# NeSC-IV/sage-icp

Measured on AMD Instinct MI355X. Metric: ICP frames/sec (120k-pt scan vs 1M-pt map), higher is better.
Workload: dtype f64

## Files before the change

### sage-icp_amd/build.py

```python
import concurrent.futures
import hashlib
import os
import subprocess

HERE = os.path.dirname(os.path.abspath(__file__))
SOURCES = ["csrc/kernels.hip", "csrc/sort.hip", "csrc/preprocess.hip", "csrc/dyn_filter.hip", "csrc/deskew.hip",
           "csrc/ingest.hip", "csrc/egress.hip", "csrc/msg.hip", "csrc/keyframe.hip", "csrc/map_update.hip",
           "csrc/map_device.hip", "csrc/capi_run.hip", "csrc/prep.hip", "csrc/capi.hip", "csrc/capi_pipeline.hip",
           "csrc/capi_outputs.hip", "csrc/caller_mem.hip", "csrc/correspond.hip"]
HEADERS = ["csrc/kernels.h", "csrc/dev_buffer.h", "csrc/sageicp_types.h", "csrc/se3_math.h", "csrc/host_map.hpp", "csrc/pipeline.hpp", "csrc/map_update.h", "csrc/egress.h", "csrc/msg.h", "csrc/metrics.hpp", "csrc/robin_order.hpp", "csrc/capi_internal.h", "csrc/prep.h", "csrc/prefetch.h", "csrc/dyn_rules.h", "csrc/probes.h", "csrc/icp_body.h", "csrc/row_shift.h", "csrc/fin_kernel.h", "csrc/loop_kernel.h", "csrc/caller_mem.h", "csrc/outputs.h", "csrc/map_device.h", "csrc/replay_pool.h", "csrc/correspond.h",
           "../include/sageicp.h"]
OUT = os.path.join(HERE, "libsageicp_hip.so")
OBJ_DIR = os.path.join(HERE, "build")

FLAGS = ["--offload-arch=gfx950", "-O3", "-std=c++17", "-fPIC", "-ffp-contract=off",
         "-Wall", "-Wextra"]


def _stamp(extra):
    h = hashlib.sha1(" ".join(FLAGS + list(extra)).encode())
    for f in HEADERS:
        with open(os.path.join(HERE, f), "rb") as fh:
            h.update(fh.read())
    return h.hexdigest()[:16]


def needs_build():
    if not os.path.exists(OUT):
        return True
    t = os.path.getmtime(OUT)
    return any(os.path.getmtime(os.path.join(HERE, f)) > t for f in SOURCES + HEADERS)


# ... 69 lines not shown
```

### sage-icp_amd/csrc/capi_internal.h

```cpp
#pragma once

#include <dlfcn.h>
#include <hip/hip_runtime.h>
#include <rccl/rccl.h>

#include <atomic>
#include <chrono>
#include <cmath>
#include <cstdio>
#include <cstdlib>
#include <cfloat>
#include <limits>
#include <memory>
#include <cstring>
#include <map>
#include <array>
#include <string>
#include <utility>
#include <vector>

#include "../../include/sageicp.h"
#include "dev_buffer.h"
#include "dyn_rules.h"
#include "host_map.hpp"
// ... 83 lines not shown

inline double now_us() {
    using namespace std::chrono;
    return duration<double, std::micro>(steady_clock::now().time_since_epoch()).count();
}

constexpr int kChunkMax = 16;

struct Scratch {
    int device = -1;
    OwnedStream stream;
    DevBuf<Point4> d_frame, d_tgt;
    DevBuf<int32_t> d_nn;
    DevBuf<Point4> d_sorted;
    DevBuf<uint32_t> d_keys, d_vals;
    DevBuf<unsigned char> d_sort_temp;
    size_t sort_cap = 0;
    DevBuf<uint32_t> d_rows;
    DevBuf<uint2> d_prev;
    DevBuf<uint32_t> d_work;
    DevBuf<double> d_partials;
    DevBuf<long long> d_acc;
    DevBuf<LoopShared> d_loop;
    unsigned long long go_word = 0;
    OwnedStream stream2;
    std::vector<uint32_t> cu_mask;
    OwnedEvent ev_solve;
    unsigned long long loop_epoch = 0;
    int num_cus = 0;
    int cu_share_i = 0, cu_share_k = 1;
    int loop_cooldown = 0;
    int loop_derate = 0;
    uint64_t calls_single_launch = 0, calls_per_iteration = 0, calls_chained = 0;
    uint32_t loop_timeouts = 0;
    int last_fallback = 0;
    DevBuf<unsigned long long> d_cand;
    DevBuf<IcpState> d_state;
    PinnedBuf<IcpState> h_state;
    PinnedBuf<IcpProgress, hipHostMallocMapped | hipHostMallocCoherent> h_prog;
    IcpProgress *d_prog = nullptr;
    std::vector<OwnedEvent> events;
    DevBuf<int32_t> d_by_query;
    DevBuf<uint32_t> d_corr_counts;
    DevBuf<unsigned long long> d_corr_words;
    PinnedBuf<unsigned long long> h_corr_words;

// ... 69 lines not shown
        return SAGEICP_OK;
    }
    int reserve_nn(size_t n) {
        if (n > d_nn.capacity()) HIPCHK(d_nn.reserve(n + n / 4 + 1024));
        return SAGEICP_OK;
    }
    int reserve_sort(size_t n) {
        if (n <= sort_cap) return SAGEICP_OK;
        sort_cap = 0;
        const size_t cap = n + n / 4 + 1024;
        HIPCHK(d_sorted.reserve(cap));
        HIPCHK(d_rows.reserve(cap * kRowWords));
        HIPCHK(d_prev.reserve(cap));
#ifdef SAGE_NN_TIMING
        HIPCHK(d_work.reserve(cap));
#endif
        HIPCHK(d_cand.reserve(2 * cap));
        HIPCHK(d_keys.reserve(2 * cap));
        HIPCHK(d_vals.reserve(2 * cap));
        HIPCHK(d_sort_temp.reserve(sort_temp_bytes(static_cast<int>(cap))));
        sort_cap = cap;
        return SAGEICP_OK;
    }
    int reserve_correspond(size_t n) {
        if (n > d_by_query.capacity()) HIPCHK(d_by_query.reserve(n + n / 4 + 1024));
        const size_t words = 2 * static_cast<size_t>(correspond_blocks(static_cast<int>(n)));
        if (words > d_corr_counts.capacity()) HIPCHK(d_corr_counts.reserve(words + words / 4 + 16));
        if (!d_corr_words) HIPCHK(d_corr_words.reserve(2));
        if (!h_corr_words) HIPCHK(h_corr_words.reserve(2));
        return SAGEICP_OK;
    }
    int reserve_partials(size_t blocks) {
        if (blocks > d_partials.capacity() / kNumSums) HIPCHK(d_partials.reserve((blocks + blocks / 4 + 256) * kNumSums));
        return SAGEICP_OK;
    }
    int reserve_events(size_t iterations) {
        while (events.size() < 5 * iterations) {
            OwnedEvent e;
            HIPCHK(e.create(hipEventDefault));
            events.push_back(std::move(e));
        }
        return SAGEICP_OK;
    }
};


// ... 91 lines not shown
```

### sage-icp_amd/csrc/capi_run.hip

```cpp
#include "capi_internal.h"

#include <condition_variable>
#include <mutex>
#include <thread>

namespace sageicp_impl {

Rccl g_rccl;
static std::mutex g_rccl_mu;


int load_rccl() {
    std::lock_guard<std::mutex> lk(g_rccl_mu);
    if (g_rccl.h) return SAGEICP_OK;
    const char *names[] = {"librccl.so.1", "librccl.so", "/opt/rocm/lib/librccl.so.1"};
    void *h = nullptr;
    for (const char *n : names) {
        h = dlopen(n, RTLD_NOW | RTLD_NOLOAD | RTLD_GLOBAL);
        if (h) break;
    }
    for (int i = 0; i < 3 && !h; ++i) h = dlopen(names[i], RTLD_NOW | RTLD_GLOBAL);
    if (!h) return fail(SAGEICP_ERR_RCCL, std::string("cannot load librccl: ") + dlerror());
    g_rccl.GetUniqueId = reinterpret_cast<decltype(g_rccl.GetUniqueId)>(dlsym(h, "ncclGetUniqueId"));
    g_rccl.CommInitRank = reinterpret_cast<decltype(g_rccl.CommInitRank)>(dlsym(h, "ncclCommInitRank"));
// ... 88 lines not shown
    ip.work = sc.d_work.data();
    ip.acc_scale = std::ldexp(1.0, -24 * std::max(acc_shift, std::min(2, std::max(0, env_int("SAGEICP_ACC_SHIFT", 0)))));
    {
        const uint64_t blocks = std::max<uint64_t>(1, (n + 3) / 4);
        int bits = 0;
        while ((1ull << bits) < blocks) ++bits;
        ip.digit_limit = std::ldexp(1.0, std::min(46, 62 - bits));
    }
    ip.counters = nullptr;
    ip.stripe_work = nullptr;
    ip.stripe_order = nullptr;
    const uint64_t qw = 64u >> lw;
    ip.nwaves = static_cast<unsigned>((n + qw - 1) / qw);
#ifdef SAGE_ICP_DELAY_PROBE
    ip.dbg_delay = static_cast<unsigned>(env_int("SAGEICP_DBG_DELAY", 0));
    ip.dbg_repeat = static_cast<unsigned>(env_int("SAGEICP_DBG_REPEAT", 0));
#endif
    return ip;
}

struct LoopPlan {
    int lw, nw, gpw, wgs;
    bool filter;
};
static int loop_wgs_per_cu(const Scratch &sc, int lw, bool filter, int nw, size_t lds) {
    static std::mutex mu;
    static std::map<std::array<long, 5>, int> cache;
    const std::array<long, 5> key{sc.device, lw, filter ? 1 : 0, nw, static_cast<long>(lds)};
    int v;
    {
        std::lock_guard<std::mutex> lk(mu);
        auto it = cache.find(key);
        if (it == cache.end()) it = cache.emplace(key, loop_blocks_per_cu(lw, filter, nw, lds)).first;
        v = it->second;
    }
    return std::min(v, SAGE_LOOP_OCC / ((nw + 3) / 4));
}
static bool plan_loop(const sageicp_map &m, uint64_t n, double sem_th, LoopPlan *out) {
    const Scratch &sc = m.sc;
    const int mode = env_int("SAGEICP_LOOP", 1);
    if (mode == 0 || n == 0 || sc.num_cus < 8) return false;
    const bool sparse = sparse_voxels(m);
    const bool filter = wants_filter(m, n, sem_th);
    const uint64_t cus = static_cast<uint64_t>(sc.num_cus);
    const int env_nw = std::min(kLoopMaxWavesHost, std::max(0, env_int("SAGEICP_LOOP_WAVES", 0)));
    const int env_gpw = std::max(0, env_int("SAGEICP_LOOP_GPW", 0));
    auto groups_at = [n](int l) { return (n + (64u >> l) - 1) / (64u >> l); };
    auto slots = [&](int k) {
        const uint64_t a = static_cast<uint64_t>(k) * cus * 15 / 16;
        int less = 0;
        for (int sh = 1; sh < sc.cu_share_k; sh *= 2) ++less;
        return (less > 0 && k > less) ? std::min(a, static_cast<uint64_t>(k - less) * cus) : a;
    };
    auto round32 = [](uint64_t w) { return std::max<uint64_t>(32, (w + 31) / 32 * 32); };
    auto countable = [](uint64_t wgs, uint64_t gpw, int lw) {
        return wgs / kLoopReplicas <= 255 && (wgs / kLoopReplicas) * gpw * ((64u >> lw) / 4u) <= 8192;
    };
    auto one_pass = [&](int lw, int nw, LoopPlan *pl) {
        const uint64_t wgs = round32((groups_at(lw) + nw - 1) / nw);
        const size_t lds = loop_lds_bytes(lw, nw, nw);
        const int k = loop_wgs_per_cu(sc, lw, filter, nw, lds);
        if (k < 1 || wgs + 32ull * static_cast<uint64_t>(sc.loop_derate) > slots(k) || !countable(wgs, nw, lw)) return false;
        *pl = LoopPlan{lw, nw, nw, static_cast<int>(wgs), filter};
        return true;
    };
    auto multi_pass = [&](int lw, LoopPlan *pl) {
        const uint64_t groups = groups_at(lw);
        int best = -1;
        const int order[] = {4, 8, 7, 6, 5, 3, 2, 1};
        for (int nw : order) {
            if (env_nw && nw != env_nw) continue;
            if (!env_nw && nw < 4) continue;
            for (int k = SAGE_LOOP_OCC / ((nw + 3) / 4); k >= 1; --k) {
                if (static_cast<uint64_t>(k) * cus < 34) break;
                uint64_t cap = slots(k) / 32 * 32;
                cap = cap > 32ull * static_cast<uint64_t>(sc.loop_derate) ? cap - 32ull * static_cast<uint64_t>(sc.loop_derate) : 0;
                if (cap < 32) continue;
                if (const int e = env_int("SAGEICP_LOOP_MAX_WGS", 0)) cap = std::min<uint64_t>(cap, static_cast<uint64_t>(e) / 32 * 32);
                uint64_t gpw = env_gpw ? static_cast<uint64_t>(env_gpw) : (groups + cap - 1) / cap;
                const uint64_t wgs = env_gpw ? round32((groups + gpw - 1) / gpw) : std::min(cap, round32(groups));
                if (wgs > cap) continue;
                if (!env_gpw) gpw = (groups + wgs - 1) / wgs;
                const size_t lds = loop_lds_bytes(lw, nw, static_cast<int>(gpw));
                if (lds > 160 * 1024 || !countable(wgs, gpw, lw)) continue;
                if (loop_wgs_per_cu(sc, lw, filter, nw, lds) < k) continue;
                if (k * nw > best) {
                    best = k * nw;
                    *pl = LoopPlan{lw, nw, static_cast<int>(gpw), static_cast<int>(wgs), filter};
                }
                break;
            }
        }
        return best > 0;
    };
    const int forced = env_int("SAGEICP_LW", -1);
    int lw = forced >= 0 ? std::min(forced, 4) : icp_lw(n, sparse);
    if (lw < 1) return false;
    if (forced < 0 && !env_gpw) {
        const uint64_t few = 15 * cus;
        if (lw < 3 && groups_at(3) <= few) lw = 3;
        if (lw == 3 && !sparse && groups_at(4) <= few) lw = 4;
        const uint64_t resident_waves = 4ull * SAGE_LOOP_OCC * cus * 15 / 16;
        while (lw > 2 && groups_at(lw) > resident_waves * 4 / 5) --lw;
    }
    const bool dbg = env_int("SAGEICP_LOOP_DEBUG", 0) != 0;
    bool ok = !env_gpw && one_pass(lw, env_nw ? env_nw : 4, out);
    if (!ok) ok = multi_pass(lw, out);
    if (dbg) {
        if (ok)
            std::fprintf(stderr, "sageicp: one-launch loop for %llu queries: %d lanes/query, %d workgroups of %d waves, <= %d units of %d queries each, "
                                 "%zu B of LDS (%d workgroups per CU by the occupancy query, %d CUs)\n",
// ... 172 lines not shown
        armed = true;
        HIPCHK(hipEventRecord(sc.ev_solve.get(), sc.stream2.get()));
        return SAGEICP_OK;
    }
    void disarm() { armed = false; }
    int send_home_now() {
        sc.go_word = epoch | 0x8000000000000000ull;
        HIPCHK(hipMemcpyAsync(&sc.d_loop.data()->go[0], &sc.go_word, sizeof(sc.go_word), hipMemcpyHostToDevice, sc.stream.get()));
        armed = false;
        return SAGEICP_OK;
    }
};

struct AttemptResult {
    bool looped = false;
    bool chain = false;
    bool chain_gave_up = false;
    int lw = 0;
    bool compact_scan = false;
    double us_nn = 0, us_fin = 0;
    uint32_t nn_launches = 0;
};

static int run_one_launch(const IcpCall &c, const AttemptPlan &p, const IcpParams &ip, const LoopParams &L,
                          SolverGuard &guard, AttemptResult &r) {
    Scratch &sc = c.sc;
    hipStream_t s = c.s;
    int rc;
    if (c.prof && (rc = sc.reserve_events(1))) return rc;
    IcpParams lp = ip;
    lp.filter = p.loop.filter ? ip.filter : 0;
    lp.nwaves = p.loop_waves;
    HIPCHK(hipMemsetAsync(sc.d_loop.data(), 0, offsetof(LoopShared, acc32), s));
    if (c.prof) HIPCHK(hipEventRecord(sc.events[1].get(), s));
    launch_loop(lp, L, p.loop.lw, s);
    if (hipPeekAtLastError() == hipSuccess) guard.disarm();
    if (c.prof) HIPCHK(hipEventRecord(sc.events[2].get(), s));
    if (solver_is_own_launch(p)) HIPCHK(hipStreamWaitEvent(s, sc.ev_solve.get(), 0));
    if ((rc = c.fetch_state(lp.nwaves))) return rc;
    const IcpState &st = *sc.h_state.data();
    r.looped = true;
    if ((st.bad_input && !c.comm) || st.exchange_failed) return SAGEICP_OK;
    if (!st.loop_aborted && st.done) {
        if (c.prof) {
            float a = 0;
            (void)hipEventElapsedTime(&a, sc.events[1].get(), sc.events[2].get());
            r.us_nn = 1e3 * a;
            r.nn_launches = static_cast<uint32_t>(std::max(1, st.iter));
        }
        return SAGEICP_OK;
    }
    r.looped = false;
    if (st.peer_aborted) {
        sc.last_fallback = SAGEICP_LOOP_FALLBACK_PEER;
    } else {
        sc.loop_cooldown = std::max(0, env_int("SAGEICP_LOOP_COOLDOWN", 256));
        if (env_int("SAGEICP_LOOP_TIMEOUT_TICKS", 0) == 0 && env_int("SAGEICP_LOOP_COUNT_TIMEOUT_RANK", -1) < 0 && sc.loop_derate < 16) ++sc.loop_derate;
        ++sc.loop_timeouts;
        sc.last_fallback = SAGEICP_LOOP_FALLBACK_TIMEOUT;
        static std::atomic<int> told{0};
        if (told.exchange(1) == 0 && env_int("SAGEICP_QUIET", 0) == 0)
            std::fprintf(stderr, "sageicp: a wait inside the one-launch ICP loop timed out (the GPU is shared with other work, or "
// ... 137 lines not shown
            const int todo = std::min(chunk, kMaxIterations - launched);
            for (int k = 0; k < todo; ++k)
                if ((rc = enqueue(k, launched + k))) return rc;
            if ((rc = c.fetch_state(ip.nwaves))) return rc;
            if (c.prof) {
                const int executed = std::min(todo, st.iter - launched);
                for (int k = 0; k < executed; ++k)
                    if (sampled(launched + k)) harvest(k);
            }
            launched += todo;
            if (st.done || launched >= kMaxIterations) return SAGEICP_OK;
            chunk = std::min(kChunkMax, chunk * 2);
        }
    }
};

static int run_attempt(const IcpCall &c, const Attempt &a, AttemptResult &r) {
    Scratch &sc = c.sc;
    int rc;
    if ((rc = c.start_state())) return rc;
    const AttemptPlan p = plan_attempt(c, a);
    if ((rc = c.m.dev.ensure_cand(wants_filter(c.m, c.n, c.sem_th), c.s))) return rc;
    if ((rc = sc.reserve_sort(c.n))) return rc;
    IcpParams ip = icp_params(c.m, sc.d_sorted.data(), c.n, c.sem_th, p.lw, a.acc_shift);
    ip.check_done = 1; ip.apply_pose = 1;
    ip.kernel = c.kernel;
    ip.accept_r2 = accept_threshold(c.max_dist);
    ip.counters = c.counting ? sc.d_cand.data() : nullptr;
    if (c.counting) HIPCHK(hipMemsetAsync(sc.d_cand.data(), 0, sizeof(unsigned long long) * 2 * (std::max(ip.nwaves, p.loop_waves) + 1), c.s));
    LoopParams L{};
    SolverGuard guard(sc);
    if (p.use_loop || p.chain) {
        if ((rc = sc.loop_streams())) return rc;
        L = solver_params(c, p, 1.0 / ip.acc_scale);
        if (solver_is_own_launch(p) && (rc = guard.start(L, c.xp))) return rc;
    }
    if ((rc = c.order_frame())) return rc;
    r = AttemptResult{};
    r.lw = p.lw;
    r.chain = p.chain;
    if (p.use_loop && (rc = run_one_launch(c, p, ip, L, guard, r))) return rc;
    r.compact_scan = r.looped ? p.loop.filter && ip.filter : ip.filter != 0;
    if (c.n > 0 && !r.looped) {
        launch_rows(ip, c.s);
        HIPCHK(hipMemsetAsync(sc.d_prev.data(), 0xFF, c.n * sizeof(uint2), c.s));
    }
    HIPCHK(hipMemsetAsync(sc.d_acc.data(), 0, sizeof(long long) * kAccReplicas * kAccWords, c.s));
    if (r.looped) return SAGEICP_OK;
    Iterations it{c, guard, r, ip, p.lw, p.chain};
    if ((rc = it.begin(L))) return rc;
    return c.polled ? it.run_polled() : it.run_chunked();
}

static void fill_stats(sageicp_stats *stats, const IcpState &st, uint64_t n, const AttemptResult &r, double us_upload, double t_begin) {
    std::memset(stats, 0, sizeof(*stats));
    stats->iterations = st.iter; stats->converged = st.converged;
    stats->n_queries = n;
    stats->n_corr_first = st.iter > 0 ? st.n_corr[0] : 0;
    stats->n_corr_last = st.iter > 0 ? st.n_corr[std::min(st.iter, kHistory) - 1] : 0;
    stats->last_step_norm = st.last_step_norm;
    stats->us_upload = us_upload;
    stats->us_nn = r.us_nn; stats->us_fin = r.us_fin;
    stats->nn_launches = r.nn_launches;
    stats->sum_candidates = st.sum_candidates; stats->pairs_evaluated = st.sum_pairs;
// ... 218 lines not shown
```

### sage-icp_amd/csrc/kernels.h

```cpp
#pragma once

#include <hip/hip_runtime.h>

#include "sageicp_types.h"

namespace sageicp {

constexpr int kRowWords = 32;
constexpr int kRowCq = 27, kRowKey = 28, kRowOcc = 31;
constexpr int kRowLdsStride = 36;

struct LoopShared;
struct IcpParams {
    const Point4 *frame;
    int n;
    const IcpState *st;
    int check_done;
    int apply_pose;
    double voxel_size;
    double inv_voxel_size;
    uint32_t *rows;
    const Slot *table;
    uint32_t mask;
    const Point4 *pts;
// ... 88 lines not shown
    IcpState *st;
    int nw;
    int gpw;
    int wgs;
    int contiguous;
    uint32_t xcd_first[9];
    unsigned long long timeout_ticks;
    unsigned long long count_timeout_ticks;
    int max_iterations;
    unsigned long long epoch;
    double T0[7];
    double acc_unscale;
    int shared_loop;
    int prio;
    int deal;
    int copies;
    int pose_map;
    IcpProgress *progress;
};
struct LoopArgs {
    IcpParams P;
    LoopParams L;
    double face_slack;
};
#ifndef SAGE_LOOP_OCC
#define SAGE_LOOP_OCC 7
#endif
constexpr int kLoopMaxWavesHost = 8;
constexpr int kLoopStripeHost = 4;
constexpr int kLoopStateWords = 24;
size_t loop_lds_bytes(int lw, int nw, int gpw);
int loop_blocks_per_cu(int lw, bool filter, int nw, size_t lds);
void launch_loop(const IcpParams &p, const LoopParams &l, int lw, hipStream_t s);
void launch_loop_solve(const LoopParams &l, const P2pParams &x, hipStream_t s);

constexpr int kMaxPartials = 1 << 16;
constexpr uint64_t kMaxQueries = (1ull << 26) - 4;

void launch_tf(Point4 *pts, int n, const IcpState *st, hipStream_t s);
void launch_scatter_points(const uint32_t *idx, const Point4 *vals, uint32_t n, Point4 *pts,
                           hipStream_t s);
void launch_scatter_slots(const uint32_t *idx, const Slot *vals, uint32_t n, Slot *table,
                          hipStream_t s);
void launch_scatter_u32(const uint32_t *idx, const uint32_t *vals, uint32_t n, uint32_t *dst, hipStream_t s);
void launch_sum_counters(const unsigned long long *c, int n, IcpState *st, hipStream_t s);

struct VdsParams {
    const Point4 *in;
    int n;
    int do_crop;
    double max_range, min_range, label_max_range;
    int n_groups;
    const int *group_counts;
    const int *group_labels;
    double group_vs[8];
    double scale;
// ... 72 lines not shown
```

### sage-icp_amd/csrc/kernels.hip

```cpp

#include <hip/hip_runtime.h>

#include <algorithm>
#include <cfloat>
#include <cstdlib>
#include <type_traits>
#include <vector>

#ifndef SAGE_ICP_STRIPE
#define SAGE_ICP_STRIPE 8
#endif
#ifndef SAGE_ICP_OCC
#define SAGE_ICP_OCC 6
#endif

#include "kernels.h"
#include "se3_math.h"
#include "sageicp_types.h"
#include "probes.h"

namespace sageicp {


template <int CTRL>
// ... 618 lines not shown
size_t loop_lds_bytes(int lw, int nw, int gpw) {
    return sizeof(uint32_t) * LoopLds<size_t>(lw, static_cast<size_t>(nw), static_cast<size_t>(gpw)).end;
}
static const void *loop_kernel(int lw, bool filter) {
#define SAGE_LOOP_K(LW_, F_) reinterpret_cast<const void *>(&k_loop<LW_, F_>)
    switch (lw) {
        case 1: return filter ? SAGE_LOOP_K(1, true) : SAGE_LOOP_K(1, false);
        case 2: return filter ? SAGE_LOOP_K(2, true) : SAGE_LOOP_K(2, false);
        case 3: return filter ? SAGE_LOOP_K(3, true) : SAGE_LOOP_K(3, false);
        case 4: return filter ? SAGE_LOOP_K(4, true) : SAGE_LOOP_K(4, false);
        default: return nullptr;
    }
#undef SAGE_LOOP_K
}
int loop_blocks_per_cu(int lw, bool filter, int nw, size_t lds) {
    if (nw < 1 || nw > kLoopMaxWaves || lds > 160 * 1024) return 0;
    const void *k = loop_kernel(lw, filter);
    if (!k) return 0;
    if (lds > 64 * 1024 && hipFuncSetAttribute(k, hipFuncAttributeMaxDynamicSharedMemorySize, 160 * 1024) != hipSuccess) return 0;
    int nb = 0;
    if (hipOccupancyMaxActiveBlocksPerMultiprocessor(&nb, k, 64 * nw, lds) != hipSuccess) return 0;
    return nb;
}
void launch_loop(const IcpParams &p, const LoopParams &l, int lw, hipStream_t s) {
    const size_t lds = loop_lds_bytes(lw, l.nw, l.gpw);
    LoopArgs a;
    a.P = p;
    a.L = l;
    a.face_slack = 1e-9 * p.voxel_size;
    void *args[] = {&a};
#ifdef SAGE_LOOP_INGRID
    (void)hipLaunchKernel(loop_kernel(lw, p.filter != 0), dim3(l.wgs + 1), dim3(64 * l.nw), args, lds, s);
#else
    (void)hipLaunchKernel(loop_kernel(lw, p.filter != 0), dim3(l.wgs), dim3(64 * l.nw), args, lds, s);
#endif
}
void launch_loop_solve(const LoopParams &l, const P2pParams &x, hipStream_t s) {
    SolveArgs a;
    a.L = l;
    a.X = x;
    if (l.copies == kChainReplicas) hipLaunchKernelGGL(k_loop_solve<kChainReplicas>, dim3(1), dim3(64), 0, s, a);
    else hipLaunchKernelGGL(k_loop_solve<kLoopReplicas>, dim3(1), dim3(64), 0, s, a);
}

int launch_gn(const GnParams &p, hipStream_t s) {
    long blocks = (static_cast<long>(p.n) + 255) / 256;
    if (blocks > 128) blocks = 128;
    if (blocks < 1) blocks = 1;
    hipLaunchKernelGGL(k_gn, dim3(static_cast<int>(blocks)), dim3(256), 0, s, p);
    return static_cast<int>(blocks);
}

// ... 11 lines not shown
```

### sage-icp_amd/csrc/loop_kernel.h

```cpp
#pragma once

namespace sageicp {


__device__ __forceinline__ int exchange_sums_wave(double *S, const P2pParams &X, unsigned long long g) {
    const int lane = static_cast<int>(threadIdx.x & 63u);
    const int slot = static_cast<int>(g & 1ull);
    const unsigned long long tag = g + 1ull;
    if (lane < kNumSums) {
        const double v = S[lane];
        for (int r = 0; r < X.nranks; ++r)
            __hip_atomic_store(&X.block[r]->sums[slot][X.rank][lane], v, __ATOMIC_RELAXED, __HIP_MEMORY_SCOPE_SYSTEM);
    }
    asm volatile("s_waitcnt vmcnt(0)" ::: "memory");
    __builtin_amdgcn_fence(__ATOMIC_RELEASE, "");
    asm volatile("s_waitcnt vmcnt(0)" ::: "memory");
    if (lane == 0)
        for (int r = 0; r < X.nranks; ++r)
            __hip_atomic_store(&X.block[r]->flag[X.rank], tag, __ATOMIC_RELAXED, __HIP_MEMORY_SCOPE_SYSTEM);
    P2pBlock *mine = X.block[X.rank];
    bool late = false, gone = false;
    if (lane < X.nranks) {
        const unsigned long long t0 = __builtin_amdgcn_s_memrealtime();
        while (__hip_atomic_load(&mine->flag[lane], __ATOMIC_RELAXED, __HIP_MEMORY_SCOPE_SYSTEM) < tag) {
// ... 282 lines not shown
        unsigned long long xg = 0ull;
        for (int it = 0;; ++it)
            if (loop_finish_iteration<kLoopReplicas>(L, X, m, it, xg)) return;
    }
#endif

    unsigned g0, gcnt;
    {
        const unsigned xcd = blockIdx.x & 7u, jb = blockIdx.x >> 3;
        const unsigned ngroups = (static_cast<unsigned>(P.n) + QW - 1u) / QW;
        unsigned lo = 0u, cnt = ngroups, idx, nwg;
        if (L.contiguous == 1) {
            lo = L.xcd_first[xcd];
            cnt = L.xcd_first[xcd + 1u] - lo;
            idx = jb;
            nwg = static_cast<unsigned>(L.wgs) >> 3;
        } else {
            idx = ((jb / kLoopStripe) * 8u + xcd) * kLoopStripe + (jb % kLoopStripe);
            nwg = static_cast<unsigned>(L.wgs);
        }
        const unsigned base = cnt / nwg, extra = cnt - base * nwg;
        g0 = lo + idx * base + min(idx, extra);
        gcnt = min(gpw, base + (idx < extra ? 1u : 0u));
    }
    constexpr unsigned BPW = QW / 4;
    const unsigned nblk_max = gpw * BPW;
    const LoopLds<unsigned> lds0(LW, static_cast<unsigned>(nw), gpw);
    uint32_t *perm0 = smem + lds0.perm;
    uint32_t *work0 = smem + lds0.work;
    uint32_t *state0 = smem + lds0.state;

    if (threadIdx.x < 9) s_pose[threadIdx.x] = P.st->R[threadIdx.x];
    else if (threadIdx.x < 12) s_pose[threadIdx.x] = P.st->T[4 + threadIdx.x - 9];
    if (threadIdx.x == 0) {
        smem[kLpArrive] = 0u;
        smem[kLpNext] = 0u;
        smem[kLpDone] = 0u;
        smem[kLpIter] = 0u;
        PROBE_LOOP_CLEAR_STATS(smem);
    }
    if (L.deal && (threadIdx.x & 63u) == 0u) {
        unsigned hw;
        asm volatile("s_getreg_b32 %0, hwreg(HW_REG_HW_ID)" : "=s"(hw));
        smem[kLpFirst + static_cast<unsigned>(wv)] = (((hw >> 4) & 3u) + (hw & 15u)) % static_cast<unsigned>(nw);
    }
    for (unsigned i = threadIdx.x; i < 2u * kWgAccWords; i += blockDim.x) smem[kLpAcc + i] = 0u;
    for (unsigned i = threadIdx.x; i < nblk_max; i += blockDim.x) {
        perm0[i] = i;
        work0[i] = 0u;
    }
    for (unsigned sl = threadIdx.x; sl < gcnt * QW; sl += blockDim.x) {
        const unsigned q = g0 * QW + sl;
        const Point4 f = P.frame[q < static_cast<unsigned>(P.n) ? q : 0u];
        {
            uint32_t *lst = state0 + sl * kLoopStateWords;
            *reinterpret_cast<Point4 *>(lst) = f;
            Point4 z;
            z.x = z.y = z.z = z.l = 0.0;
            *reinterpret_cast<Point4 *>(lst + 8) = z;
            *reinterpret_cast<uint4 *>(lst + kStPrev) = make_uint4(0xFFFFFFFFu, 0u, static_cast<uint32_t>(kNoVoxel),
                                                                   static_cast<uint32_t>(kNoVoxel));
            *reinterpret_cast<uint4 *>(lst + kStPrev + 4) = make_uint4(static_cast<uint32_t>(kNoVoxel), 0u, 0u, 0u);
        }
    }
    __syncthreads();
    if (L.deal) {
        unsigned claimed = 0u, kept = 0u, table[kLoopMaxWaves];
        for (int w2 = 0; w2 < nw; ++w2) {
            const unsigned pr = smem[kLpFirst + static_cast<unsigned>(w2)];
            table[w2] = pr;
            if (!((claimed >> pr) & 1u)) { claimed |= 1u << pr; kept |= 1u << w2; }
        }
        for (int w2 = 0; w2 < nw; ++w2)
            if (!((kept >> w2) & 1u)) {
                const unsigned pr = static_cast<unsigned>(__builtin_ctz(~claimed));
                table[w2] = pr;
                claimed |= 1u << pr;
            }
        __syncthreads();
        if (threadIdx.x == 0) {
            for (int w2 = 0; w2 < nw; ++w2) smem[kLpFirst + static_cast<unsigned>(w2)] = table[w2];
            smem[kLpNext] = static_cast<unsigned>(nw);
        }
        __syncthreads();
    }
// ... 155 lines not shown
```

Measured before the change: 248.2.

## Deal loop-kernel query groups to workgroups by estimated cost via prefix-sum partition

Adds a unit-deal scheme that assigns query groups to persistent loop-kernel workgroups through a table of first indices instead of an even split. The default mode 2 builds the table on the host once, using uniform costs and optional per-workgroup weights, and caches it across calls. Mode 1 runs a rows kernel, a per-unit cost kernel and a single-block scan kernel on device before the loop, and the loop then preloads rows and voxel keys into LDS. The aim is to reduce tail imbalance across workgroups, at the cost of an extra table read per workgroup and, in mode 1, extra small launches.

```diff
diff --git a/sage-icp_amd/build.py b/sage-icp_amd/build.py
--- a/sage-icp_amd/build.py
+++ b/sage-icp_amd/build.py
@@ -7,8 +7,8 @@
 SOURCES = ["csrc/kernels.hip", "csrc/sort.hip", "csrc/preprocess.hip", "csrc/dyn_filter.hip", "csrc/deskew.hip",
            "csrc/ingest.hip", "csrc/egress.hip", "csrc/msg.hip", "csrc/keyframe.hip", "csrc/map_update.hip",
            "csrc/map_device.hip", "csrc/capi_run.hip", "csrc/prep.hip", "csrc/capi.hip", "csrc/capi_pipeline.hip",
-           "csrc/capi_outputs.hip", "csrc/caller_mem.hip", "csrc/correspond.hip"]
-HEADERS = ["csrc/kernels.h", "csrc/dev_buffer.h", "csrc/sageicp_types.h", "csrc/se3_math.h", "csrc/host_map.hpp", "csrc/pipeline.hpp", "csrc/map_update.h", "csrc/egress.h", "csrc/msg.h", "csrc/metrics.hpp", "csrc/robin_order.hpp", "csrc/capi_internal.h", "csrc/prep.h", "csrc/prefetch.h", "csrc/dyn_rules.h", "csrc/probes.h", "csrc/icp_body.h", "csrc/row_shift.h", "csrc/fin_kernel.h", "csrc/loop_kernel.h", "csrc/caller_mem.h", "csrc/outputs.h", "csrc/map_device.h", "csrc/replay_pool.h", "csrc/correspond.h",
+           "csrc/capi_outputs.hip", "csrc/caller_mem.hip", "csrc/correspond.hip", "csrc/unit_deal.hip"]
+HEADERS = ["csrc/kernels.h", "csrc/dev_buffer.h", "csrc/sageicp_types.h", "csrc/se3_math.h", "csrc/host_map.hpp", "csrc/pipeline.hpp", "csrc/map_update.h", "csrc/egress.h", "csrc/msg.h", "csrc/metrics.hpp", "csrc/robin_order.hpp", "csrc/capi_internal.h", "csrc/prep.h", "csrc/prefetch.h", "csrc/dyn_rules.h", "csrc/probes.h", "csrc/icp_body.h", "csrc/row_shift.h", "csrc/fin_kernel.h", "csrc/loop_kernel.h", "csrc/caller_mem.h", "csrc/outputs.h", "csrc/map_device.h", "csrc/replay_pool.h", "csrc/correspond.h", "csrc/unit_deal.h",
            "../include/sageicp.h"]
 OUT = os.path.join(HERE, "libsageicp_hip.so")
 OBJ_DIR = os.path.join(HERE, "build")
diff --git a/sage-icp_amd/csrc/capi_internal.h b/sage-icp_amd/csrc/capi_internal.h
--- a/sage-icp_amd/csrc/capi_internal.h
+++ b/sage-icp_amd/csrc/capi_internal.h
@@ -129,6 +129,9 @@
     DevBuf<double> d_partials;
     DevBuf<long long> d_acc;
     DevBuf<LoopShared> d_loop;
+    DevBuf<uint32_t> d_deal;
+    DevBuf<uint64_t> d_deal_cum;
+    std::array<uint32_t, 6> deal_key{};
     unsigned long long go_word = 0;
     OwnedStream stream2;
     std::vector<uint32_t> cu_mask;
@@ -244,6 +247,12 @@
         sort_cap = cap;
         return SAGEICP_OK;
     }
+    int reserve_deal(size_t units, size_t wgs) {
+        const size_t words = units + 2 * (wgs + 1) + 1 + wgs;
+        if (words > d_deal.capacity()) HIPCHK(d_deal.reserve(words + words / 4 + 64));
+        if (2 * (units + 1) > d_deal_cum.capacity()) HIPCHK(d_deal_cum.reserve(2 * (units + units / 4 + 64)));
+        return SAGEICP_OK;
+    }
     int reserve_correspond(size_t n) {
         if (n > d_by_query.capacity()) HIPCHK(d_by_query.reserve(n + n / 4 + 1024));
         const size_t words = 2 * static_cast<size_t>(correspond_blocks(static_cast<int>(n)));
diff --git a/sage-icp_amd/csrc/capi_run.hip b/sage-icp_amd/csrc/capi_run.hip
--- a/sage-icp_amd/csrc/capi_run.hip
+++ b/sage-icp_amd/csrc/capi_run.hip
@@ -1,4 +1,5 @@
 #include "capi_internal.h"
+#include "unit_deal.h"
 
 #include <condition_variable>
 #include <mutex>
@@ -134,6 +135,7 @@
 struct LoopPlan {
     int lw, nw, gpw, wgs;
     bool filter;
+    bool multi;
 };
 static int loop_wgs_per_cu(const Scratch &sc, int lw, bool filter, int nw, size_t lds) {
     static std::mutex mu;
@@ -173,7 +175,7 @@
         const size_t lds = loop_lds_bytes(lw, nw, nw);
         const int k = loop_wgs_per_cu(sc, lw, filter, nw, lds);
         if (k < 1 || wgs + 32ull * static_cast<uint64_t>(sc.loop_derate) > slots(k) || !countable(wgs, nw, lw)) return false;
-        *pl = LoopPlan{lw, nw, nw, static_cast<int>(wgs), filter};
+        *pl = LoopPlan{lw, nw, nw, static_cast<int>(wgs), filter, false};
         return true;
     };
     auto multi_pass = [&](int lw, LoopPlan *pl) {
@@ -198,7 +200,7 @@
                 if (loop_wgs_per_cu(sc, lw, filter, nw, lds) < k) continue;
                 if (k * nw > best) {
                     best = k * nw;
-                    *pl = LoopPlan{lw, nw, static_cast<int>(gpw), static_cast<int>(wgs), filter};
+                    *pl = LoopPlan{lw, nw, static_cast<int>(gpw), static_cast<int>(wgs), filter, true};
                 }
                 break;
             }
@@ -417,7 +419,97 @@
     uint32_t nn_launches = 0;
 };
 
-static int run_one_launch(const IcpCall &c, const AttemptPlan &p, const IcpParams &ip, const LoopParams &L,
+struct DealPlan {
+    int mode = 0;
+    uint32_t units = 0, wgs = 0, gpw = 0, light = 0, alpha = 100;
+    uint32_t *cost = nullptr, *want = nullptr, *first = nullptr, *kind = nullptr, *weight = nullptr;
+    uint64_t *cum = nullptr, *cumf = nullptr;
+};
+static DealPlan deal_plan(Scratch &sc, const AttemptPlan &p) {
+    DealPlan d;
+    const int mode = env_int("SAGEICP_LOOP_BALANCE", 2);
+    if (mode <= 0 || !p.use_loop || !p.loop.multi || p.loop_waves > unitdeal::kMaxUnits ||
+        static_cast<uint64_t>(p.loop_waves) > static_cast<uint64_t>(p.loop.wgs) * static_cast<uint64_t>(p.loop.gpw) ||
+        env_int("SAGEICP_LOOP_CONTIGUOUS", 0) != 0)
+        return d;
+    d.mode = mode >= 2 ? 2 : 1;
+    d.units = p.loop_waves;
+    d.wgs = static_cast<uint32_t>(p.loop.wgs);
+    d.gpw = static_cast<uint32_t>(p.loop.gpw);
+    d.alpha = static_cast<uint32_t>(std::min(100, std::max(0, env_int("SAGEICP_LOOP_ALPHA", 0))));
+    const int light = env_int("SAGEICP_LOOP_LIGHT", -1);
+    if (light >= 0) d.light = std::min(d.wgs, static_cast<uint32_t>(light));
+    else if (sc.num_cus > 0 && d.wgs >= static_cast<uint32_t>(sc.num_cus)) d.light = d.wgs % static_cast<uint32_t>(sc.num_cus);
+    if (d.alpha == 100) d.light = 0;
+    return d;
+}
+static void deal_place(Scratch &sc, DealPlan &d) {
+    d.cost = sc.d_deal.data();
+    d.want = d.cost + d.units;
+    d.first = d.want + d.wgs + 1;
+    d.kind = d.first + d.wgs + 1;
+    d.weight = d.kind + 1;
+    d.cum = sc.d_deal_cum.data();
+    d.cumf = d.cum + d.units + 1;
+}
+static std::vector<uint32_t> deal_weights(const DealPlan &d) {
+    std::vector<uint32_t> w(d.wgs, 100u);
+    for (uint32_t j = d.wgs - d.light; j < d.wgs; ++j) w[j] = d.alpha;
+    return w;
+}
+static int deal_prepare(Scratch &sc, DealPlan &d) {
+    if (!d.mode) return SAGEICP_OK;
+    const uint32_t *before = sc.d_deal.data();
+    if (int rc = sc.reserve_deal(d.units, d.wgs)) return rc;
+    deal_place(sc, d);
+    const std::array<uint32_t, 6> key{static_cast<uint32_t>(d.mode), d.units, d.wgs, d.gpw, d.light, d.alpha};
+    if (before == sc.d_deal.data() && key == sc.deal_key) return SAGEICP_OK;
+    sc.deal_key = {};
+    const std::vector<uint32_t> w = deal_weights(d);
+    std::vector<uint32_t> up(2 * static_cast<size_t>(d.wgs) + 2, 0u);
+    std::copy(w.begin(), w.end(), up.begin() + d.wgs + 2);
+    if (d.mode == 2) {
+        const std::vector<uint32_t> cost(d.units, 1u);
+        std::vector<uint64_t> cum(d.units + 1), cumf(d.units + 1);
+        up[d.wgs + 1] = unitdeal::deal(cost.data(), d.units, d.light ? w.data() : nullptr, d.wgs, d.gpw, cum.data(), cumf.data(), up.data()) == 1 ? 1u : 0u;
+    }
+    HIPCHK(hipMemcpy(d.first, up.data(), sizeof(uint32_t) * up.size(), hipMemcpyHostToDevice));
+    sc.deal_key = key;
+    return SAGEICP_OK;
+}
+static void report_deal(const DealPlan &d) {
+    const uint32_t wgs = d.wgs, gpw = d.gpw;
+    std::vector<uint32_t> cost(d.units, 1u), first(wgs + 1), host(wgs + 1);
+    std::vector<uint64_t> cum(d.units + 1), cumf(d.units + 1);
+    uint32_t kind = 0;
+    if ((d.mode == 1 && hipMemcpy(cost.data(), d.cost, sizeof(uint32_t) * d.units, hipMemcpyDeviceToHost) != hipSuccess) ||
+        hipMemcpy(first.data(), d.first, sizeof(uint32_t) * (wgs + 1), hipMemcpyDeviceToHost) != hipSuccess ||
+        hipMemcpy(&kind, d.kind, sizeof(uint32_t), hipMemcpyDeviceToHost) != hipSuccess) {
+        (void)hipGetLastError();
+        return;
+    }
+    const std::vector<uint32_t> w = deal_weights(d);
+    const int hk = unitdeal::deal(cost.data(), d.units, d.light ? w.data() : nullptr, wgs, gpw, cum.data(), cumf.data(), host.data());
+    uint32_t lo = 0xFFFFFFFFu, hi = 0u, moved = 0u;
+    uint64_t light_units = 0;
+    for (uint32_t j = 0; j < wgs; ++j) {
+        lo = std::min(lo, first[j + 1] - first[j]);
+        hi = std::max(hi, first[j + 1] - first[j]);
+        if (first[j] != unitdeal::even_first(j, d.units, wgs) || first[j + 1] != unitdeal::even_first(j + 1, d.units, wgs)) ++moved;
+        if (j >= wgs - d.light) light_units += first[j + 1] - first[j];
+    }
+    const uint64_t heavy = unitdeal::heaviest(cum.data(), first.data(), wgs), even = unitdeal::heaviest_even(cum.data(), d.units, wgs);
+    std::fprintf(stderr, "sageicp: one-launch loop: %u units dealt by %s to %u workgroups: min %u, mean %.2f, max %u units per workgroup, %u ranges "
+                         "unlike the even deal's (%s; heaviest workgroup %llu against %llu under the even deal, mean %.1f; the host's deal is %s); "
+                         "the last %u workgroups at %u %%: %llu units\n",
+                 d.units, d.mode == 1 ? "work" : "weight", wgs, lo, static_cast<double>(d.units) / wgs, hi, moved,
+                 kind ? "the table by cost" : "the even deal: the table was heavier",
+                 static_cast<unsigned long long>(heavy), static_cast<unsigned long long>(even), static_cast<double>(cum[d.units]) / wgs,
+                 (hk == static_cast<int>(kind) && host == first) ? "the same" : "DIFFERENT", d.light, d.alpha,
+                 static_cast<unsigned long long>(light_units));
+}
+
+static int run_one_launch(const IcpCall &c, const AttemptPlan &p, const IcpParams &ip, const LoopParams &L, const DealPlan &deal,
                           SolverGuard &guard, AttemptResult &r) {
     Scratch &sc = c.sc;
     hipStream_t s = c.s;
@@ -427,12 +519,19 @@
     lp.filter = p.loop.filter ? ip.filter : 0;
     lp.nwaves = p.loop_waves;
     HIPCHK(hipMemsetAsync(sc.d_loop.data(), 0, offsetof(LoopShared, acc32), s));
+    if (deal.mode == 1) {
+        launch_rows(lp, s);
+        launch_unit_cost(lp.rows, lp.n, p.loop.lw, deal.cost, s);
+        launch_deal_units(deal.cost, deal.light ? deal.weight : nullptr, deal.units, deal.wgs, deal.gpw, deal.cum, deal.cumf, deal.want,
+                          deal.first, deal.kind, s);
+    }
     if (c.prof) HIPCHK(hipEventRecord(sc.events[1].get(), s));
-    launch_loop(lp, L, p.loop.lw, s);
+    launch_loop(lp, L, p.loop.lw, deal.mode == 1, deal.mode ? deal.first : nullptr, s);
     if (hipPeekAtLastError() == hipSuccess) guard.disarm();
     if (c.prof) HIPCHK(hipEventRecord(sc.events[2].get(), s));
     if (solver_is_own_launch(p)) HIPCHK(hipStreamWaitEvent(s, sc.ev_solve.get(), 0));
     if ((rc = c.fetch_state(lp.nwaves))) return rc;
+    if (deal.mode && env_int("SAGEICP_LOOP_DEBUG", 0) != 0) report_deal(deal);
     const IcpState &st = *sc.h_state.data();
     r.looped = true;
     if ((st.bad_input && !c.comm) || st.exchange_failed) return SAGEICP_OK;
@@ -616,6 +715,8 @@
     const AttemptPlan p = plan_attempt(c, a);
     if ((rc = c.m.dev.ensure_cand(wants_filter(c.m, c.n, c.sem_th), c.s))) return rc;
     if ((rc = sc.reserve_sort(c.n))) return rc;
+    DealPlan deal = deal_plan(sc, p);
+    if ((rc = deal_prepare(sc, deal))) return rc;
     IcpParams ip = icp_params(c.m, sc.d_sorted.data(), c.n, c.sem_th, p.lw, a.acc_shift);
     ip.check_done = 1; ip.apply_pose = 1;
     ip.kernel = c.kernel;
@@ -633,7 +734,7 @@
     r = AttemptResult{};
     r.lw = p.lw;
     r.chain = p.chain;
-    if (p.use_loop && (rc = run_one_launch(c, p, ip, L, guard, r))) return rc;
+    if (p.use_loop && (rc = run_one_launch(c, p, ip, L, deal, guard, r))) return rc;
     r.compact_scan = r.looped ? p.loop.filter && ip.filter : ip.filter != 0;
     if (c.n > 0 && !r.looped) {
         launch_rows(ip, c.s);
diff --git a/sage-icp_amd/csrc/kernels.h b/sage-icp_amd/csrc/kernels.h
--- a/sage-icp_amd/csrc/kernels.h
+++ b/sage-icp_amd/csrc/kernels.h
@@ -134,6 +134,8 @@
     IcpParams P;
     LoopParams L;
     double face_slack;
+    int rows_built;
+    const uint32_t *first;
 };
 #ifndef SAGE_LOOP_OCC
 #define SAGE_LOOP_OCC 7
@@ -143,7 +145,10 @@
 constexpr int kLoopStateWords = 24;
 size_t loop_lds_bytes(int lw, int nw, int gpw);
 int loop_blocks_per_cu(int lw, bool filter, int nw, size_t lds);
-void launch_loop(const IcpParams &p, const LoopParams &l, int lw, hipStream_t s);
+void launch_loop(const IcpParams &p, const LoopParams &l, int lw, bool rows_built, const uint32_t *first, hipStream_t s);
+void launch_unit_cost(const uint32_t *rows, int n, int lw, uint32_t *cost, hipStream_t s);
+void launch_deal_units(const uint32_t *cost, const uint32_t *weight, uint32_t units, uint32_t wgs, uint32_t gpw, uint64_t *cum,
+                       uint64_t *cumf, uint32_t *want, uint32_t *first, uint32_t *kind, hipStream_t s);
 void launch_loop_solve(const LoopParams &l, const P2pParams &x, hipStream_t s);
 
 constexpr int kMaxPartials = 1 << 16;
diff --git a/sage-icp_amd/csrc/kernels.hip b/sage-icp_amd/csrc/kernels.hip
--- a/sage-icp_amd/csrc/kernels.hip
+++ b/sage-icp_amd/csrc/kernels.hip
@@ -664,12 +664,14 @@
     if (hipOccupancyMaxActiveBlocksPerMultiprocessor(&nb, k, 64 * nw, lds) != hipSuccess) return 0;
     return nb;
 }
-void launch_loop(const IcpParams &p, const LoopParams &l, int lw, hipStream_t s) {
+void launch_loop(const IcpParams &p, const LoopParams &l, int lw, bool rows_built, const uint32_t *first, hipStream_t s) {
     const size_t lds = loop_lds_bytes(lw, l.nw, l.gpw);
     LoopArgs a;
     a.P = p;
     a.L = l;
     a.face_slack = 1e-9 * p.voxel_size;
+    a.rows_built = rows_built ? 1 : 0;
+    a.first = l.contiguous == 1 ? nullptr : first;
     void *args[] = {&a};
 #ifdef SAGE_LOOP_INGRID
     (void)hipLaunchKernel(loop_kernel(lw, p.filter != 0), dim3(l.wgs + 1), dim3(64 * l.nw), args, lds, s);
diff --git a/sage-icp_amd/csrc/loop_kernel.h b/sage-icp_amd/csrc/loop_kernel.h
--- a/sage-icp_amd/csrc/loop_kernel.h
+++ b/sage-icp_amd/csrc/loop_kernel.h
@@ -328,6 +328,10 @@
         const unsigned base = cnt / nwg, extra = cnt - base * nwg;
         g0 = lo + idx * base + min(idx, extra);
         gcnt = min(gpw, base + (idx < extra ? 1u : 0u));
+        if (A.first) {
+            g0 = static_cast<unsigned>(__builtin_amdgcn_readfirstlane(static_cast<int>(A.first[idx])));
+            gcnt = min(gpw, static_cast<unsigned>(__builtin_amdgcn_readfirstlane(static_cast<int>(A.first[idx + 1u]))) - g0);
+        }
     }
     constexpr unsigned BPW = QW / 4;
     const unsigned nblk_max = gpw * BPW;
@@ -364,9 +368,20 @@
             Point4 z;
             z.x = z.y = z.z = z.l = 0.0;
             *reinterpret_cast<Point4 *>(lst + 8) = z;
-            *reinterpret_cast<uint4 *>(lst + kStPrev) = make_uint4(0xFFFFFFFFu, 0u, static_cast<uint32_t>(kNoVoxel),
-                                                                   static_cast<uint32_t>(kNoVoxel));
-            *reinterpret_cast<uint4 *>(lst + kStPrev + 4) = make_uint4(static_cast<uint32_t>(kNoVoxel), 0u, 0u, 0u);
+            uint4 key = make_uint4(static_cast<uint32_t>(kNoVoxel), static_cast<uint32_t>(kNoVoxel), static_cast<uint32_t>(kNoVoxel), 0u);
+            if (A.rows_built && q < static_cast<unsigned>(P.n)) key = *reinterpret_cast<const uint4 *>(P.rows + static_cast<size_t>(q) * kRowWords + kRowKey);
+            *reinterpret_cast<uint4 *>(lst + kStPrev) = make_uint4(0xFFFFFFFFu, 0u, key.x, key.y);
+            *reinterpret_cast<uint4 *>(lst + kStPrev + 4) = make_uint4(key.z, key.w, 0u, 0u);
+        }
+    }
+    if (A.rows_built) {
+        uint32_t *rows0 = smem + lds0.rows;
+        for (unsigned i = threadIdx.x; i < gcnt * QW * 8u; i += blockDim.x) {
+            const unsigned sl = i >> 3, piece = i & 7u;
+            const unsigned q = g0 * QW + sl;
+            if (piece < 7u && q < static_cast<unsigned>(P.n))
+                *reinterpret_cast<uint4 *>(rows0 + sl * kRowLdsStride + 4u * piece) =
+                    *reinterpret_cast<const uint4 *>(P.rows + static_cast<size_t>(q) * kRowWords + 4u * piece);
         }
     }
     __syncthreads();
diff --git a/sage-icp_amd/csrc/unit_deal.h b/sage-icp_amd/csrc/unit_deal.h
--- /dev/null
+++ b/sage-icp_amd/csrc/unit_deal.h
@@ -0,0 +1,160 @@
+#pragma once
+
+#include <stdint.h>
+
+#if defined(__HIPCC__) || defined(__CUDACC__)
+#define SAGE_UD_HD __host__ __device__ __forceinline__
+#else
+#define SAGE_UD_HD inline
+#endif
+
+namespace sageicp {
+namespace unitdeal {
+
+constexpr uint32_t kMaxUnits = 1u << 20;
+constexpr uint32_t kCostFixed = 5500u;
+constexpr uint32_t kCostPerPoint = 1u;
+constexpr uint32_t kMaxCost = (1u << 22) - 1u;
+constexpr uint32_t kMaxWeight = 1u << 10;
+
+SAGE_UD_HD uint32_t unit_cost(uint64_t est) {
+    const uint64_t c = static_cast<uint64_t>(kCostFixed) + static_cast<uint64_t>(kCostPerPoint) * est;
+    return c < kMaxCost ? static_cast<uint32_t>(c) : kMaxCost;
+}
+
+constexpr int kFloorSteps = 8;
+SAGE_UD_HD uint32_t floor_next(uint32_t tau, uint64_t total, uint64_t below, uint64_t sum_below, uint64_t room) {
+    const uint64_t have = total + below * tau - sum_below, need = static_cast<uint64_t>(tau) * room;
+    if (have <= need) return tau;
+    const uint64_t slope = room - below;
+    return tau + static_cast<uint32_t>((have - need + slope - 1u) / slope);
+}
+
+SAGE_UD_HD uint32_t even_first(uint32_t j, uint32_t units, uint32_t wgs) {
+    const uint32_t base = units / wgs, extra = units - base * wgs;
+    return j * base + (j < extra ? j : extra);
+}
+
+SAGE_UD_HD uint64_t share(uint64_t total, uint64_t wcum, uint64_t wtot) { return total * wcum / wtot; }
+
+SAGE_UD_HD uint32_t nearest(const uint64_t *cum, uint32_t units, uint64_t t) {
+    uint32_t lo = 0u, hi = units;
+    while (lo < hi) {
+        const uint32_t mid = lo + (hi - lo) / 2u;
+        if (cum[mid] < t) lo = mid + 1u;
+        else hi = mid;
+    }
+    if (lo > 0u && (cum[lo] < t || t - cum[lo - 1u] <= cum[lo] - t)) {
+        const uint64_t v = cum[lo - 1u];
+        uint32_t a = 0u, b = lo - 1u;
+        while (a < b) {
+            const uint32_t mid = a + (b - a) / 2u;
+            if (cum[mid] < v) a = mid + 1u;
+            else b = mid;
+        }
+        return a;
+    }
+    return lo;
+}
+
+SAGE_UD_HD uint32_t want(uint32_t near, uint32_t j, uint32_t units, uint32_t wgs, uint32_t gpw) {
+    const uint64_t room = static_cast<uint64_t>(wgs - j) * gpw;
+    const uint32_t least = room >= units ? 0u : units - static_cast<uint32_t>(room);
+    return near > least ? near : least;
+}
+
+struct Carry {
+    int64_t add, floor;
+};
+constexpr int64_t kNoFloor = -(1ll << 60);
+SAGE_UD_HD Carry carry_identity() { return Carry{0, kNoFloor}; }
+SAGE_UD_HD Carry carry_step(uint32_t wanted, uint32_t gpw) {
+    return Carry{static_cast<int64_t>(wanted) - static_cast<int64_t>(gpw), 0};
+}
+SAGE_UD_HD int64_t carry_apply(const Carry &f, int64_t x) { return x + f.add > f.floor ? x + f.add : f.floor; }
+SAGE_UD_HD Carry compose(const Carry &first, const Carry &then) {
+    const int64_t m = first.floor + then.add;
+    return Carry{first.add + then.add, m > then.floor ? m : then.floor};
+}
+
+inline uint32_t floor_cost(const uint32_t *cost, uint32_t units, uint32_t wgs, uint32_t gpw, bool *reached = nullptr) {
+    uint64_t total = 0u;
+    for (uint32_t u = 0; u < units; ++u) total += cost[u] < kMaxCost ? cost[u] : kMaxCost;
+    uint32_t tau = 0u;
+    for (int k = 0; k < kFloorSteps; ++k) {
+        uint64_t below = 0u, sum_below = 0u;
+        for (uint32_t u = 0; u < units; ++u) {
+            const uint32_t c = cost[u] < kMaxCost ? cost[u] : kMaxCost;
+            if (c < tau) {
+                ++below;
+                sum_below += c;
+            }
+        }
+        const uint32_t next = floor_next(tau, total, below, sum_below, static_cast<uint64_t>(wgs) * gpw);
+        if (next == tau) {
+            if (reached) *reached = true;
+            return tau;
+        }
+        tau = next;
+    }
+    if (reached) *reached = false;
+    return tau;
+}
+
+inline bool deal_by_cost(const uint32_t *cost, uint32_t units, const uint32_t *weight, uint32_t wgs, uint32_t gpw,
+                         uint64_t *cum, uint64_t *cumf, uint32_t *first) {
+    if (wgs == 0u || units > kMaxUnits || static_cast<uint64_t>(wgs) * gpw < units) return false;
+    const uint32_t tau = floor_cost(cost, units, wgs, gpw);
+    cum[0] = 0u;
+    cumf[0] = 0u;
+    for (uint32_t u = 0; u < units; ++u) {
+        const uint32_t c = cost[u] < kMaxCost ? cost[u] : kMaxCost;
+        cum[u + 1u] = cum[u] + c;
+        cumf[u + 1u] = cumf[u] + (c > tau ? c : tau);
+    }
+    uint64_t wtot = 0u;
+    if (weight)
+        for (uint32_t j = 0; j < wgs; ++j) wtot += weight[j] < kMaxWeight ? weight[j] : kMaxWeight;
+    const bool equal = !weight || wtot == 0u;
+    if (equal) wtot = wgs;
+    uint64_t wcum = 0u;
+    uint32_t before = 0u;
+    Carry run = carry_identity();
+    first[0] = 0u;
+    for (uint32_t j = 1; j <= wgs; ++j) {
+        wcum += equal ? 1u : (weight[j - 1u] < kMaxWeight ? weight[j - 1u] : kMaxWeight);
+        const uint32_t w = j == wgs ? units : want(nearest(cumf, units, share(cumf[units], wcum, wtot)), j, units, wgs, gpw);
+        run = compose(run, carry_step(w - before, gpw));
+        first[j] = w - static_cast<uint32_t>(carry_apply(run, 0));
+        before = w;
+    }
+    return true;
+}
+
+inline uint64_t heaviest(const uint64_t *cum, const uint32_t *first, uint32_t wgs) {
+    uint64_t m = 0u;
+    for (uint32_t j = 0; j < wgs; ++j) {
+        const uint64_t c = cum[first[j + 1u]] - cum[first[j]];
+        if (c > m) m = c;
+    }
+    return m;
+}
+inline uint64_t heaviest_even(const uint64_t *cum, uint32_t units, uint32_t wgs) {
+    uint64_t m = 0u;
+    for (uint32_t j = 0; j < wgs; ++j) {
+        const uint64_t c = cum[even_first(j + 1u, units, wgs)] - cum[even_first(j, units, wgs)];
+        if (c > m) m = c;
+    }
+    return m;
+}
+
+inline int deal(const uint32_t *cost, uint32_t units, const uint32_t *weight, uint32_t wgs, uint32_t gpw, uint64_t *cum,
+                uint64_t *cumf, uint32_t *first) {
+    if (!deal_by_cost(cost, units, weight, wgs, gpw, cum, cumf, first)) return -1;
+    if (heaviest(cum, first, wgs) <= heaviest_even(cum, units, wgs)) return 1;
+    for (uint32_t j = 0; j <= wgs; ++j) first[j] = even_first(j, units, wgs);
+    return 0;
+}
+
+}
+}
diff --git a/sage-icp_amd/csrc/unit_deal.hip b/sage-icp_amd/csrc/unit_deal.hip
--- /dev/null
+++ b/sage-icp_amd/csrc/unit_deal.hip
@@ -0,0 +1,164 @@
+#include <hip/hip_runtime.h>
+
+#include "kernels.h"
+#include "unit_deal.h"
+
+namespace sageicp {
+
+namespace ud = unitdeal;
+
+__global__ __launch_bounds__(256) void k_unit_cost(const uint32_t *rows, uint32_t n, uint32_t qw, uint32_t units, uint32_t *cost) {
+    const uint32_t u = blockIdx.x * 256u + threadIdx.x;
+    if (u >= units) return;
+    const uint32_t q0 = u * qw, q1 = min(q0 + qw, n);
+    uint64_t est = 0u;
+    for (uint32_t q = q0; q < q1; ++q) est += rows[static_cast<size_t>(q) * kRowWords + kRowCq];
+    cost[u] = ud::unit_cost(est);
+}
+
+constexpr unsigned kDealThreads = 1024;
+
+template <typename T, typename Op>
+__device__ __forceinline__ T deal_scan(T v, T identity, T *lds, Op op, T *all) {
+    const unsigned t = threadIdx.x;
+    lds[t] = v;
+    __syncthreads();
+    for (unsigned d = 1; d < kDealThreads; d <<= 1) {
+        const T later = lds[t];
+        const T earlier = t >= d ? lds[t - d] : identity;
+        __syncthreads();
+        lds[t] = op(earlier, later);
+        __syncthreads();
+    }
+    const T before = t ? lds[t - 1u] : identity;
+    *all = lds[kDealThreads - 1u];
+    __syncthreads();
+    return before;
+}
+
+struct DealArgs {
+    const uint32_t *cost;
+    const uint32_t *weight;
+    uint32_t units, wgs, gpw;
+    uint64_t *cum;
+    uint64_t *cumf;
+    uint32_t *want;
+    uint32_t *first;
+    uint32_t *kind;
+};
+
+__global__ __launch_bounds__(kDealThreads) void k_deal_units(DealArgs A) {
+    __shared__ ud::Carry s_carry[kDealThreads];
+    __shared__ unsigned long long s_max[2];
+    uint64_t *s_u64 = reinterpret_cast<uint64_t *>(s_carry);
+    const unsigned t = threadIdx.x;
+    const uint32_t units = A.units, wgs = A.wgs, gpw = A.gpw;
+    auto add = [](uint64_t a, uint64_t b) { return a + b; };
+    auto clampc = [](uint32_t c) { return c < ud::kMaxCost ? c : ud::kMaxCost; };
+    auto clampw = [](uint32_t w) { return w < ud::kMaxWeight ? w : ud::kMaxWeight; };
+
+    const uint32_t per = (units + kDealThreads - 1u) / kDealThreads;
+    const uint32_t u0 = min(t * per, units), u1 = min(u0 + per, units);
+    uint64_t mine = 0u, true_total;
+    for (uint32_t u = u0; u < u1; ++u) mine += clampc(A.cost[u]);
+    uint64_t run = deal_scan<uint64_t>(mine, 0u, s_u64, add, &true_total);
+    for (uint32_t u = u0; u < u1; ++u) {
+        A.cum[u] = run;
+        run += clampc(A.cost[u]);
+    }
+    if (t == 0u) A.cum[units] = true_total;
+
+    uint32_t tau = 0u;
+    for (int k = 0; k < ud::kFloorSteps; ++k) {
+        unsigned long long below = 0ull, sum_below = 0ull;
+        for (uint32_t u = u0; u < u1; ++u) {
+            const uint32_t c = clampc(A.cost[u]);
+            if (c < tau) {
+                ++below;
+                sum_below += c;
+            }
+        }
+        if (t < 2u) s_max[t] = 0ull;
+        __syncthreads();
+        if (below) {
+            atomicAdd(&s_max[0], below);
+            atomicAdd(&s_max[1], sum_below);
+        }
+        __syncthreads();
+        const uint32_t next = ud::floor_next(tau, true_total, s_max[0], s_max[1], static_cast<uint64_t>(wgs) * gpw);
+        __syncthreads();
+        if (next == tau) break;
+        tau = next;
+    }
+    mine = 0u;
+    for (uint32_t u = u0; u < u1; ++u) mine += max(clampc(A.cost[u]), tau);
+    uint64_t total;
+    run = deal_scan<uint64_t>(mine, 0u, s_u64, add, &total);
+    for (uint32_t u = u0; u < u1; ++u) {
+        A.cumf[u] = run;
+        run += max(clampc(A.cost[u]), tau);
+    }
+    if (t == 0u) A.cumf[units] = total;
+
+    const uint32_t perw = (wgs + kDealThreads - 1u) / kDealThreads;
+    const uint32_t j0 = min(t * perw, wgs), j1 = min(j0 + perw, wgs);
+    uint64_t wmine = 0u, wtot;
+    if (A.weight)
+        for (uint32_t j = j0; j < j1; ++j) wmine += clampw(A.weight[j]);
+    uint64_t wrun = deal_scan<uint64_t>(wmine, 0u, s_u64, add, &wtot);
+    const bool equal = !A.weight || wtot == 0u;
+    if (equal) {
+        wtot = wgs;
+        wrun = j0;
+    }
+    if (t == 0u) A.want[0] = 0u;
+    for (uint32_t j = j0; j < j1; ++j) {
+        wrun += equal ? 1u : clampw(A.weight[j]);
+        A.want[j + 1u] = j + 1u == wgs ? units : ud::want(ud::nearest(A.cumf, units, ud::share(total, wrun, wtot)), j + 1u, units, wgs, gpw);
+    }
+    __syncthreads();
+
+    ud::Carry f = ud::carry_identity(), all;
+    for (uint32_t j = j0; j < j1; ++j) f = ud::compose(f, ud::carry_step(A.want[j + 1u] - A.want[j], gpw));
+    ud::Carry before = deal_scan<ud::Carry>(f, ud::carry_identity(), s_carry,
+                                            [](const ud::Carry &a, const ud::Carry &b) { return ud::compose(a, b); }, &all);
+    if (t == 0u) {
+        A.first[0] = 0u;
+        s_max[0] = 0ull;
+        s_max[1] = 0ull;
+    }
+    for (uint32_t j = j0; j < j1; ++j) {
+        before = ud::compose(before, ud::carry_step(A.want[j + 1u] - A.want[j], gpw));
+        A.first[j + 1u] = A.want[j + 1u] - static_cast<uint32_t>(ud::carry_apply(before, 0));
+    }
+    __syncthreads();
+
+    unsigned long long mt = 0ull, me = 0ull;
+    for (uint32_t j = j0; j < j1; ++j) {
+        const uint64_t ct = A.cum[A.first[j + 1u]] - A.cum[A.first[j]];
+        const uint64_t ce = A.cum[ud::even_first(j + 1u, units, wgs)] - A.cum[ud::even_first(j, units, wgs)];
+        mt = ct > mt ? ct : mt;
+        me = ce > me ? ce : me;
+    }
+    atomicMax(&s_max[0], mt);
+    atomicMax(&s_max[1], me);
+    __syncthreads();
+    const bool keep = s_max[0] <= s_max[1];
+    if (!keep)
+        for (uint32_t j = j0; j < j1; ++j) A.first[j + 1u] = ud::even_first(j + 1u, units, wgs);
+    if (t == 0u) *A.kind = keep ? 1u : 0u;
+}
+
+void launch_unit_cost(const uint32_t *rows, int n, int lw, uint32_t *cost, hipStream_t s) {
+    const uint32_t qw = 64u >> lw, units = (static_cast<uint32_t>(n) + qw - 1u) / qw;
+    if (units == 0u) return;
+    hipLaunchKernelGGL(k_unit_cost, dim3((units + 255u) / 256u), dim3(256), 0, s, rows, static_cast<uint32_t>(n), qw, units, cost);
+}
+
+void launch_deal_units(const uint32_t *cost, const uint32_t *weight, uint32_t units, uint32_t wgs, uint32_t gpw, uint64_t *cum,
+                       uint64_t *cumf, uint32_t *want, uint32_t *first, uint32_t *kind, hipStream_t s) {
+    DealArgs a{cost, weight, units, wgs, gpw, cum, cumf, want, first, kind};
+    hipLaunchKernelGGL(k_deal_units, dim3(1), dim3(kDealThreads), 0, s, a);
+}
+
+}
```

Result: faster. 254.0 (median of 5 runs) (+2.3%).
